# gchq/annchor

Hardware: AMD Instinct MI355X
Metric: knn_graph_builds_per_s (1 / Annchor.fit() wall-clock; BASELINE: k-NN graph build time + recall@k) (higher is better)
Workload: dtype int32 bit-vectors (Levenshtein) + f64 (bounds/regression/selection); 1 GPU; load_strings Levenshtein N=1600 n_anchors=15 k=25 p_work=0.12 niters=2; parallelism=one GPU

## Files before the change

annchor_amd/_native.py:

```python
import ctypes
import os

import numpy as np

_HERE = os.path.dirname(os.path.abspath(__file__))
LIB_PATH = os.environ.get("ANNCHOR_HIP_LIB", os.path.join(_HERE, "libannchor_hip.so"))

F_D, F_A, F_SID, F_IJS, F_I_PTR, F_I_IDX, F_FEATURES, F_NCM, F_RA, F_LABELS, F_THRESH, F_PROB, F_CAND, F_NEXT, F_DAD = range(1, 16)
_FIELD_DTYPE = {
    F_D: np.float64, F_A: np.int64, F_SID: np.uint64, F_IJS: np.int64, F_I_PTR: np.int64, F_I_IDX: np.int64,
    F_FEATURES: np.float64, F_NCM: np.uint8, F_RA: np.float64, F_LABELS: np.int64, F_THRESH: np.float64,
    F_PROB: np.float64, F_CAND: np.int64, F_NEXT: np.int64, F_DAD: np.float64,
}

METRIC_LEVENSHTEIN, METRIC_EUCLIDEAN_F32, METRIC_EUCLIDEAN_F64, METRIC_WASSERSTEIN = 1, 2, 3, 4
METRIC_COSINE_F32, METRIC_COSINE_F64 = 5, 6
METRIC_DTW_F32, METRIC_DTW_F64 = 7, 8
METRIC_FRECHET_F32, METRIC_FRECHET_F64 = 9, 10
METRIC_HAUSDORFF_F32, METRIC_HAUSDORFF_F64 = 11, 12
METRIC_ERP_F32, METRIC_ERP_F64 = 13, 14
METRIC_EMD_POINTS_F32, METRIC_EMD_POINTS_F64 = 15, 16
METRIC_JACCARD_TOKENS, METRIC_JACCARD_BITS = 17, 18
METRIC_WEIGHTED_LEVENSHTEIN = 19
METRIC_MSM_F32, METRIC_MSM_F64 = 20, 21
# ... 80 lines not shown
    "annchor_legacy_prefetch": (ctypes.c_int, [ctypes.c_uint32, _i64]),
    "annchor_legacy_generate": (ctypes.c_int, [ctypes.c_uint32, _i64]),
    "annchor_legacy_generate_at_next_wait": (ctypes.c_int, [_vp, ctypes.c_uint32, _i64, _i64]),
    "annchor_legacy_choice_ranks": (ctypes.c_int, [ctypes.c_uint32, _vp, _vp, _i32, _vp, _vp]),
    "annchor_legacy_choice_begin": (ctypes.c_int, [ctypes.c_uint32, _vp, _vp, _i32, ctypes.POINTER(_vp)]),
    "annchor_legacy_choice_end": (ctypes.c_int, [_vp, _vp, _vp]),
    "annchor_ols_bins": (ctypes.c_int, [_vp, _vp, _vp, _i64, _i32, _vp, _i32, _vp, _vp, _vp, _vp]),
    "annchor_gather_features": (ctypes.c_int, [_vp, _vp, _i64, _vp]),
    "annchor_evaluate_samples": (ctypes.c_int, [_vp, _vp, _i64, _vp]),
    "annchor_set_samples": (ctypes.c_int, [_vp, _vp, _i64, _vp]),
    "annchor_predict_merge": (ctypes.c_int, [_vp, _vp, _i32, _vp, _vp, _i32, _i32, _vp]),
    "annchor_merge_host_prediction": (ctypes.c_int, [_vp, _vp, _i32, _i32]),
    "annchor_set_labels": (ctypes.c_int, [_vp, _vp]),
    "annchor_select_candidates": (ctypes.c_int, [_vp, _i32, _i32, _vp, _vp, _i32, _i64, _i32,
                                                 ctypes.POINTER(_i64), ctypes.POINTER(_i64)]),
    "annchor_select_prepare": (ctypes.c_int, [_vp, _i32, _i32]),
    "annchor_mark_candidates": (ctypes.c_int, [_vp]),
    "annchor_refine_candidates": (ctypes.c_int, [_vp]),
    "annchor_park_refine": (ctypes.c_int, [_vp, _i32]),
    "annchor_set_refined": (ctypes.c_int, [_vp, _vp, _i64]),
    "annchor_update_bounds": (ctypes.c_int, [_vp]),
    "annchor_update_bounds_prepare": (ctypes.c_int, [_vp]),
    "annchor_overlap_stats": (ctypes.c_int, [_vp, _vp]),
    "annchor_neighbor_graph": (ctypes.c_int, [_vp, _i32, _vp, _vp]),
    "annchor_stream_bind": (ctypes.c_int, [_vp, _vp, _i64, _i32, _i64, _i32]),
    "annchor_stream_anchor_round": (ctypes.c_int, [_vp, _vp, _i32, _i32, ctypes.POINTER(_dbl), ctypes.POINTER(_i64)]),
    "annchor_stream_get_row": (ctypes.c_int, [_vp, _i64, _vp]),
    "annchor_stream_order": (ctypes.c_int, [_vp, _i32] + [ctypes.POINTER(_vp)] * 6 + [ctypes.POINTER(_i64), ctypes.POINTER(_i32),
                                                                                   ctypes.POINTER(_i32)]),
    "annchor_stream_knn": (ctypes.c_int, [_vp, _vp, _vp, _vp, _vp, _vp, _vp, _i64, _i32, _i32, _i32, _i32, _i32, _i32, _dbl, _i32, _i32, _vp,
                                          _vp, _vp, ctypes.POINTER(_i64)]),
    "annchor_stream_knn_begin": (ctypes.c_int, [_vp, _vp, _vp, _vp, _vp, _vp, _vp, _i64, _i32, _i32, _i32, _i32, _i32, _i32, _i32,
                                                ctypes.POINTER(_vp), ctypes.POINTER(_i64)]),
    "annchor_stream_knn_join": (ctypes.c_int, [_vp, _vp, _i32, ctypes.POINTER(_vp), ctypes.POINTER(_i64)]),
    "annchor_stream_join_rev_begin": (ctypes.c_int, [_vp, _vp, ctypes.POINTER(_vp), ctypes.POINTER(_vp), ctypes.POINTER(_i64)]),
    "annchor_stream_order_begin": (ctypes.c_int, [_vp, _i32, _i32, _i32, ctypes.POINTER(_vp), ctypes.POINTER(_vp), ctypes.POINTER(_i64)]),
    "annchor_stream_order_end": (ctypes.c_int, [_vp] + [ctypes.POINTER(_vp)] * 6 + [ctypes.POINTER(_i64), ctypes.POINTER(_i32),
                                                                                       ctypes.POINTER(_i32)]),
    "annchor_stream_last_counts": (ctypes.c_int, [_vp, ctypes.POINTER(_i64), ctypes.POINTER(_i64)]),
    "annchor_stream_last_kernel": (ctypes.c_int, [_vp, ctypes.POINTER(ctypes.c_int32), ctypes.POINTER(_i64)]),
    "annchor_stream_last_tile_kernels": (ctypes.c_int, [_vp, ctypes.POINTER(ctypes.c_int32), ctypes.POINTER(ctypes.c_int32)]),
    "annchor_stream_budget": (ctypes.c_int, [_i32, _dbl, _i32, ctypes.POINTER(_i32), ctypes.POINTER(_i32), ctypes.POINTER(_i32)]),
    "annchor_stream_knn_end": (ctypes.c_int, [_vp, _vp, _vp, _vp, ctypes.POINTER(_i64)]),
    "annchor_stream_knn_run": (ctypes.c_int, [_vp, _vp, _vp, _vp, _vp, _vp, _vp, _i64, _i32, _i32, _i32, _i32, _i32, _i32, _dbl, _i32, _i32,
                                               ctypes.POINTER(_i64)]),
    "annchor_stream_knn_fetch": (ctypes.c_int, [_vp, _vp, _vp, _vp]),
# ... 652 lines not shown
        self._chk(self.lib.annchor_mark_candidates(self.h))

    def refine_candidates(self):
        self._chk(self.lib.annchor_refine_candidates(self.h))

    def park_refine(self, action):
        self._chk(self.lib.annchor_park_refine(self.h, int(action)))

    def set_refined(self, exact):
        exact = _c(exact, np.float64)
        self._chk(self.lib.annchor_set_refined(self.h, _ptr(exact), len(exact)))

    def update_bounds(self):
        self._chk(self.lib.annchor_update_bounds(self.h))

    def update_bounds_prepare(self):
        self._chk(self.lib.annchor_update_bounds_prepare(self.h))

    def overlap_stats(self):
        out = np.zeros(2, dtype=np.int64)
        self._chk(self.lib.annchor_overlap_stats(self.h, _ptr(out)))
        return bool(out[0]), int(out[1])

    def neighbor_graph(self, k):
        idx = np.zeros((self.nx, k), dtype=np.int64)
        dist = np.zeros((self.nx, k), dtype=np.float64)
        self._chk(self.lib.annchor_neighbor_graph(self.h, int(k), _ptr(idx), _ptr(dist)))
        return idx, dist

    def stream_bind(self, X, global_base=0, device_ptr=None, shape=None):
        if device_ptr is not None:
            n, d = shape
            self._chk(self.lib.annchor_stream_bind(self.h, device_ptr, int(n), int(d), int(global_base), 1))
        else:
            X = _c(X, np.float32)
            n, d = X.shape
            self._chk(self.lib.annchor_stream_bind(self.h, _ptr(X), n, d, int(global_base), 0))
        self.nx, self.metric = int(n), METRIC_EUCLIDEAN_F32
        self._stream_dim = int(d)

    def stream_bind_f64(self, X, global_base=0, centre=None):
        X = _c(X, np.float64)
        n, d = X.shape
        cin = _c(centre, np.float64) if centre is not None else None
        if cin is not None and cin.shape != (d,):
            raise ValueError("centre must be float64 [%d]" % d)
# ... 361 lines not shown
```

annchor_amd/csrc/common.h:

```cpp
#pragma once
#include <hip/hip_runtime.h>

#include <cstdint>
#include <cstdio>
#include <cstring>
#include <string>
#include <vector>
#include <chrono>

#include "../../include/annchor_hip.h"

#define ANN_WAVE 64

struct DevBuf {
    void *p = nullptr;
    size_t cap = 0;
    bool in_arena = false;
    template <typename T> T *as() const { return reinterpret_cast<T *>(p); }
};

struct ProfEntry {
    const char *name;
    double ms = 0;
    int64_t launches = 0;
// ... 105 lines not shown

    DevBuf lb, ub, dad, RA, prob;
    DevBuf anc, ncm, label;
    bool have_features = false, have_RA = false;
    int64_t n_unc = -1;
    int64_t n_unc_after_features = -1;

    DevBuf spos, sy;
    DevBuf draw_J, draw_next, draw_q1;
    DevBuf sfeat, spred;
    int64_t sfeat_rows = 0;
    DevBuf model;
    DevBuf ols_scratch;
    std::vector<DevBuf *> own_allocs;
    int prof_group_entry = -1;
    bool model_fitted = false;
    bool errs_on_device = false;
    int model_nb = 0;
    DevBuf dev_flags;
    bool dev_flags_clean = false;
    bool gn_err_clean = false;
    bool state_prewarmed = false;
    DevBuf sstats;
    DevBuf hs_key, hs_pos, hs_misc;
    int64_t nsamp = 0;

    DevBuf thresh;
    DevBuf cand, next;
    int64_t ncand = 0, nnext = 0;
    bool cand_marked = false;
    DevBuf gl_val, gl_pos, gl_cnt, gl_ncomp, marked, markcount;
    DevBuf gn_state;
    bool sel_prepared = false;
    int sel_k = 0, sel_nmin = 0;
    bool gn_pending = false;
    int gn_round = 0, gn_L = 0;
    DevBuf sel_hist, sel_state, blk_cnt, blk_off;
    DevBuf sel_pass_state;
    DevBuf tie_lists, tie_hist;
    const void *tie_hist_clean = nullptr;
    DevBuf sel2, sel_bufA, sel_bufB, sel_seg;
    const void *sel2_clean = nullptr;
    DevBuf errs, errptr;
    DevBuf ecdf_index;
    DevBuf cptr, cidx, cval;
    DevBuf c16, cbnd;
// ... 31 lines not shown
        }                                                                                       \
    } while (0)

#define ANN_TRY(expr)                \
    do {                             \
        int _r = (expr);             \
        if (_r != ANNCHOR_OK) return _r; \
    } while (0)

#define ANN_REQUIRE(c, cond, code, ...)    \
    do {                                   \
        if (!(cond)) {                     \
            ann_set_err((c), __VA_ARGS__); \
            return (code);                 \
        }                                  \
    } while (0)

int ann_reserve(annchor_ctx *c, DevBuf &b, size_t bytes);
int ann_arena_init(annchor_ctx *c, int64_t nx);
int ann_prewarm_state(annchor_ctx *c);
void ann_lev_ap_probe(annchor_ctx *c);
size_t ann_sel2_table_bytes();
size_t ann_tie_hist_bytes();
size_t ann_sel_state_bytes();
int ann_h2d(annchor_ctx *c, void *dst, const void *src, size_t bytes);
hipError_t ann_sync(annchor_ctx *c, const char *where);
int ann_dev_alloc(annchor_ctx *c, void **p, size_t want, size_t *got);
void ann_dev_free(annchor_ctx *c, void *p, size_t bytes);
struct Sel2Epilogue;
int ann_kth_async(annchor_ctx *c, const double *vals, const uint8_t *flag, int64_t n, const int64_t *ks, int nk,
                  const unsigned long long **d_prefix, const int **d_unfinished, const Sel2Epilogue *epi = nullptr);
void ann_kth_async_done(annchor_ctx *c);
int ann_d2h(annchor_ctx *c, void *dst, const void *src, size_t bytes);
int ann_d2h_then(annchor_ctx *c, void *dst, const void *src, size_t bytes, int (*then)(annchor_ctx *));
int ann_d2h2(annchor_ctx *c, void *dst1, const void *src1, size_t bytes1, void *dst2, const void *src2, size_t bytes2);

int ann_prof_entry(annchor_ctx *c, const char *name);
struct ProfGroup {
    annchor_ctx *c;
    int entry = -1;
    hipEvent_t a = nullptr, b = nullptr;
    ProfGroup(annchor_ctx *ctx, const char *name);
    ~ProfGroup();
};

struct ProfScope {
// ... 172 lines not shown
```

annchor_amd/csrc/ctx.hip:

```cpp
#include <cstdarg>
#include <cmath>
#include <cstdlib>

#include "common.h"
#include <algorithm>
#include <chrono>
#include <mutex>

static std::string g_create_err;
void ann_stream_release(annchor_ctx *c);
void ann_enemies_release(annchor_ctx *c);
void ann_draw_forget(annchor_ctx *c);
void ann_comm_release(annchor_ctx *c);
hipError_t ann_comm_guarded_sync(annchor_ctx *c, hipStream_t stream, const char *where);

const char *ann_set_err(annchor_ctx *c, const char *fmt, ...)
{
    char buf[1024];
    va_list ap;
    va_start(ap, fmt);
    vsnprintf(buf, sizeof buf, fmt, ap);
    va_end(ap);
    if (c && c->comm_aborted && c->err.rfind("collective timed out", 0) == 0) return c->err.c_str();
    if (c) c->err = buf; else g_create_err = buf;
// ... 127 lines not shown
    size_t bytes = (size_t)(pairs * 112.0) + (size_t)nx * 4096 + ((size_t)64 << 20);
    if (c->arena) {
        if (c->arena_size >= bytes || c->arena_off != 0) return ANNCHOR_OK;
        ann_dev_free(c, c->arena, c->arena_size);
        c->arena = nullptr;
        c->arena_size = 0;
    }
    void *p = nullptr;
    size_t got = 0;
    if ((p = pool_take(c->device, bytes, &got)) != nullptr) bytes = got;
    else if (hipMalloc(&p, bytes) != hipSuccess) { (void)hipGetLastError(); return ANNCHOR_OK; }
    c->arena = (char *)p;
    c->arena_size = bytes;
    c->arena_off = 0;
    return ANNCHOR_OK;
}

int ann_prewarm_state(annchor_ctx *c)
{
    if (!c->arena || c->state_prewarmed) return ANNCHOR_OK;
    const size_t slot_bytes = sizeof(unsigned long long) * 4 * 1024 + 64;
    struct Piece { DevBuf *b; size_t bytes; };
    Piece pieces[] = {{&c->dev_flags, sizeof(int32_t) * 16}, {&c->lev_cursors, 4 * sizeof(int32_t)}, {&c->sel_state, ann_sel_state_bytes()},
                      {&c->sel2, ann_sel2_table_bytes()},    {&c->tie_hist, ann_tie_hist_bytes()},   {&c->lev_ap, slot_bytes}};
    size_t need = 0;
    for (auto &q : pieces) {
        if (q.b->p) return ANNCHOR_OK;
        need += (q.bytes + 255) & ~(size_t)255;
    }
    if (c->arena_off + need > c->arena_size) return ANNCHOR_OK;
    char *first = c->arena + c->arena_off;
    for (auto &q : pieces) ANN_TRY(ann_reserve(c, *q.b, q.bytes));
    ANN_CHECK_HIP(c, hipMemsetAsync(first, 0, need, c->stream));
    c->dev_flags_clean = true;
    c->lev_cursor_epoch = 0;
    c->gn_err_clean = true;
    c->sel2_clean = c->sel2.p;
    c->tie_hist_clean = c->tie_hist.p;
    c->lev_ap_epoch = 0;
    c->state_prewarmed = true;
    return ANNCHOR_OK;
}

int ann_h2d(annchor_ctx *c, void *dst, const void *src, size_t bytes)
{
    if (bytes == 0) return ANNCHOR_OK;
    if (c->pin && bytes <= annchor_ctx::PIN_SLOT_BYTES) {
        const int sl = c->pin_next;
        c->pin_next = (sl + 1) % annchor_ctx::PIN_SLOTS;
        if (c->pin_busy[sl]) ANN_CHECK_HIP(c, hipEventSynchronize(c->pin_ev[sl]));
        unsigned char *slot = c->pin + (size_t)sl * annchor_ctx::PIN_SLOT_BYTES;
        memcpy(slot, src, bytes);
        ANN_CHECK_HIP(c, hipMemcpyAsync(dst, slot, bytes, hipMemcpyHostToDevice, c->stream));
        ANN_CHECK_HIP(c, hipEventRecord(c->pin_ev[sl], c->stream));
        c->pin_busy[sl] = true;
        return ANNCHOR_OK;
    }
    ANN_CHECK_HIP(c, hipMemcpyAsync(dst, src, bytes, hipMemcpyHostToDevice, c->stream));
    ANN_CHECK_HIP(c, ann_sync(c, __func__));
    return ANNCHOR_OK;
}
// ... 227 lines not shown
}

int ann_side_join(annchor_ctx *c)
{
    if (!c->side_pending) return ANNCHOR_OK;
    c->side_pending = false;
    ANN_CHECK_HIP(c, hipStreamWaitEvent(c->main_stream, c->side_done_ev, 0));
    return ANNCHOR_OK;
}

SideScope::SideScope(annchor_ctx *ctx) : c(ctx) { c->stream = c->side_stream; }
SideScope::~SideScope()
{
    (void)hipEventRecord(c->side_done_ev, c->side_stream);
    c->side_pending = true;
    c->stream = c->main_stream;
}

extern "C" int annchor_overlap_stats(annchor_ctx *c, int64_t *out)
{
    if (!c || !out) return ANNCHOR_EINVAL;
    out[0] = c->overlap_parts != 0 && c->side_stream != nullptr;
    out[1] = c->ub_prepared_taken;
    return ANNCHOR_OK;
}

extern "C" int annchor_create(int device, annchor_ctx **out)
{
    if (!out) return ANNCHOR_EINVAL;
    *out = nullptr;
    int count = 0;
    hipError_t e = hipGetDeviceCount(&count);
    if (e != hipSuccess || count <= 0) {
        ann_set_err(nullptr, "no HIP device available (%s)", e == hipSuccess ? "count = 0" : hipGetErrorString(e));
        return ANNCHOR_ENODEV;
    }
    if (device < 0 || device >= count) {
        ann_set_err(nullptr, "device %d out of range (have %d)", device, count);
        return ANNCHOR_EINVAL;
    }
    annchor_ctx *c = new annchor_ctx();
    c->device = device;
    if ((e = hipSetDevice(device)) != hipSuccess) {
        ann_set_err(nullptr, "device init failed: %s", hipGetErrorString(e));
        delete c;
        return ANNCHOR_EHIP;
// ... 961 lines not shown
```

annchor_amd/csrc/features.hip:

```cpp
#include "common.h"
#include "selstate.h"
#include <mutex>

#pragma clang fp contract(off)

__global__ __launch_bounds__(256) void k_features(const int2 *__restrict__ ij, int64_t n, const double *__restrict__ Dt,
                                                 int64_t nx, int na, const int32_t *__restrict__ cA,
                                                 const int32_t *__restrict__ anchorRank, double *__restrict__ lb,
                                                 double *__restrict__ ub, double *__restrict__ dad,
                                                 uint8_t *__restrict__ anc, uint8_t *__restrict__ ncm)
{
    int64_t p = (int64_t)blockIdx.x * blockDim.x + threadIdx.x;
    if (p >= n) return;
    const int2 q = ij[p];
    const int i = q.x, j = q.y;
    double l = 0.0, u = INFINITY;
    const int i0 = __builtin_amdgcn_readfirstlane(i);
    if (__all(i == i0)) {
        for (int a0 = 0; a0 < na; a0 += 8) {
            double di[8], dj[8];
#pragma unroll
            for (int e = 0; e < 8; ++e) {
                const size_t row = (size_t)min(a0 + e, na - 1) * nx;
                di[e] = Dt[row + i0];
// ... 416 lines not shown
    }
    __syncthreads();
    if ((int)threadIdx.x < be.nb) {
        unsigned long long s = 0;
        for (int w = 0; w < BC_THREADS / 64; ++w) s += lc[w][threadIdx.x];
        if (s) atomicAdd(&counts[threadIdx.x], s);
    }
}
__global__ __launch_bounds__(BC_THREADS) void k_bin_counts(const double *__restrict__ dad, const uint8_t *__restrict__ ncm,
                                                          int64_t n, BinEdges be, unsigned long long *__restrict__ counts)
{
    bin_counts_body(dad, ncm, n, be, counts);
}

__global__ __launch_bounds__(BC_THREADS) void k_bin_counts_dev(const double *__restrict__ dad, const uint8_t *__restrict__ ncm,
                                                              int64_t n, SamplerStats *__restrict__ st)
{
    __shared__ BinEdges be;
    if (threadIdx.x == 0) be = st->be;
    __syncthreads();
    bin_counts_body(dad, ncm, n, be, st->counts);
}

static int load_bins(annchor_ctx *c, const double *bins, int32_t nbins, BinEdges &be);

__host__ __device__ __forceinline__ unsigned long long ann_splitmix64(unsigned long long x)
{
    x += 0x9E3779B97F4A7C15ull;
    x = (x ^ (x >> 30)) * 0xBF58476D1CE4E5B9ull;
    x = (x ^ (x >> 27)) * 0x94D049BB133111EBull;
    return x ^ (x >> 31);
}

#define HS_CAP 4096
struct HsParams {
    unsigned long long seed_key;
    unsigned long long thr[MAXBINS];
};

#define HS_U 8
__global__ __launch_bounds__(256) void k_hs_collect(const double *__restrict__ dad, const uint8_t *__restrict__ ncm, int64_t n,
                                                   BinEdges be, HsParams hp, unsigned long long *__restrict__ lkey,
                                                   int32_t *__restrict__ lpos, uint32_t *__restrict__ lcnt)
{
    __shared__ double se[MAXBINS + 1];
    __shared__ unsigned long long sthr[MAXBINS];
// ... 166 lines not shown
    for (int k = 0; k <= nbins; ++k) be.e[k] = bins[k];
    return ANNCHOR_OK;
}

extern "C" int annchor_bin_counts(annchor_ctx *c, const double *bins, int32_t nbins, int64_t *counts)
{
    if (!c || !bins || !counts) return ANNCHOR_EINVAL;
    ANN_REQUIRE(c, c->have_features, ANNCHOR_EINVAL, "features not computed");
    ANN_CHECK_HIP(c, hipSetDevice(c->device));
    BinEdges be;
    ANN_TRY(load_bins(c, bins, nbins, be));
    ANN_TRY(ann_reserve(c, c->tmp2, 8 * MAXBINS));
    ANN_CHECK_HIP(c, hipMemsetAsync(c->tmp2.p, 0, 8 * MAXBINS, c->stream));
    const int64_t ntiles = (c->n + BC_TILE - 1) / BC_TILE;
    const int blocks = (int)(ntiles <= 256 ? ntiles : std::min<int64_t>(1024, std::max<int64_t>(256, ntiles / 4)));
    {
        ProfScope ps(c, "sampler_bin_counts", (double)c->n * 9.0);
        k_bin_counts<<<blocks, BC_THREADS, 0, c->stream>>>(c->dad.as<double>(), c->ncm.as<uint8_t>(), c->n, be,
                                                   c->tmp2.as<unsigned long long>());
    }
    return ann_d2h(c, counts, c->tmp2.p, 8 * (size_t)nbins);
}

extern "C" int annchor_sampler_stats(annchor_ctx *c, const int64_t *ks, int32_t n_partitions, double *q, double *edges,
                                     int64_t *counts, int32_t *fused)
{
    if (!c || !ks || !q || !edges || !counts || !fused) return ANNCHOR_EINVAL;
    ANN_REQUIRE(c, c->have_features, ANNCHOR_EINVAL, "features not computed");
    ANN_REQUIRE(c, n_partitions >= 2 && n_partitions <= MAXBINS, ANNCHOR_ELIMIT, "2..%d partitions supported", MAXBINS);
    ANN_CHECK_HIP(c, hipSetDevice(c->device));
    *fused = 0;
    const unsigned long long *d_prefix = nullptr;
    const int *d_unfinished = nullptr;
    ANN_TRY(ann_reserve(c, c->sstats, sizeof(SamplerStats)));
    SamplerStats *st = c->sstats.as<SamplerStats>();
    {
        Sel2Epilogue ep;
        memset(&ep, 0, sizeof ep);
        ep.kind = 1; ep.st = st; ep.nparts = n_partitions;
        ANN_TRY(ann_kth_async(c, c->dad.as<double>(), c->ncm.as<uint8_t>(), c->n, ks, 2, &d_prefix, &d_unfinished, &ep));
    }
    if (d_prefix) {
        const int64_t ntiles = (c->n + BC_TILE - 1) / BC_TILE;
        const int blocks = (int)(ntiles <= 256 ? ntiles : std::min<int64_t>(1024, std::max<int64_t>(256, ntiles / 4)));
        {
            ProfScope ps(c, "sampler_bin_counts", (double)c->n * 9.0);
            k_bin_counts_dev<<<blocks, BC_THREADS, 0, c->stream>>>(c->dad.as<double>(), c->ncm.as<uint8_t>(), c->n, st);
        }
        ANN_CHECK_HIP(c, hipGetLastError());
        SamplerStats h;
        if (c->park_refine) {
            c->park_refine = false;
            ANN_TRY(ann_d2h_then(c, &h, st, sizeof h, ann_refine_released));
        } else
        ANN_TRY(ann_d2h(c, &h, st, sizeof h));
        const int unfinished = h.unfinished;
        ann_kth_async_done(c);
        if (!unfinished) {
            q[0] = h.q[0]; q[1] = h.q[1];
            for (int b = 0; b <= n_partitions; ++b) edges[b] = h.be.e[b];
            for (int b = 0; b < n_partitions; ++b) counts[b] = (int64_t)h.counts[b];
            *fused = 1;
            return ANNCHOR_OK;
        }
    }
    return ann_kth_smallest(c, c->dad.as<double>(), c->ncm.as<uint8_t>(), c->n, ks, 2, q);
}

#define RB_THREADS 256
#define RB_ITEMS 8
#define RB_TILE (RB_THREADS * RB_ITEMS)

__global__ __launch_bounds__(RB_THREADS) void k_rb_count(const double *__restrict__ dad, const uint8_t *__restrict__ ncm,
                                                        int64_t n, BinEdges be, uint32_t *__restrict__ blkcnt)
{
    __shared__ unsigned int lc[MAXBINS];
    for (int t = threadIdx.x; t < MAXBINS; t += blockDim.x) lc[t] = 0;
    __syncthreads();
    int64_t base = (int64_t)blockIdx.x * RB_TILE;
    double v[RB_ITEMS];
// ... 1084 lines not shown
```

annchor_amd/csrc/scan.hip:

```cpp
#include "common.h"
#include "selstate.h"

#define SCAN_THREADS 256
#define SCAN_ITEMS 8
#define SCAN_TILE (SCAN_THREADS * SCAN_ITEMS)

__device__ __forceinline__ int64_t block_exclusive_scan_i64(int64_t v, int64_t *total)
{
    __shared__ int64_t wsum[SCAN_THREADS / 64];
    const int lane = threadIdx.x & 63, wave = threadIdx.x >> 6;
    int64_t inc = v;
#pragma unroll
    for (int off = 1; off < 64; off <<= 1) {
        int64_t o = __shfl_up(inc, off);
        if (lane >= off) inc += o;
    }
    if (lane == 63) wsum[wave] = inc;
    __syncthreads();
    int64_t base = 0, tot = 0;
#pragma unroll
    for (int w = 0; w < SCAN_THREADS / 64; ++w) {
        if (w < wave) base += wsum[w];
        tot += wsum[w];
    }
// ... 175 lines not shown
        if (threadIdx.x == 0) { o->nq = nq; o->vor = st_prev->vor; o->vand = st_prev->vand; }
    }
    if (pass == 8) return;
    const int shift = 56 - 8 * pass;
    if ((((st_prev->vor ^ st_prev->vand) >> shift) & 0xffull) == 0) return;
    uint32_t *hist = hist_all + (size_t)pass * SEL_MAXQ * 256;
    for (int t = threadIdx.x; t < SEL_MAXQ * 256; t += blockDim.x) lh[t] = 0;
    uint64_t pre[SEL_MAXQ];
    for (int q = 0; q < SEL_MAXQ; ++q) pre[q] = q < nq ? sh.prefix[q] : 0;
    __syncthreads();
    const uint64_t himask = shift == 56 ? 0ull : (~0ull << (shift + 8));
    for (int64_t t = (int64_t)blockIdx.x * blockDim.x + threadIdx.x; t < n; t += (int64_t)gridDim.x * blockDim.x) {
        if (flag && !flag[t]) continue;
        uint64_t key = ann_key_asc(vals[t]);
        uint32_t d = (uint32_t)(key >> shift) & 0xffu;
        for (int q = 0; q < nq; ++q)
            if ((key & himask) == (pre[q] & himask)) atomicAdd(&lh[q * 256 + d], 1u);
    }
    __syncthreads();
    for (int t = threadIdx.x; t < nq * 256; t += blockDim.x)
        if (lh[t]) atomicAdd(&hist[t], lh[t]);
}

#define S2_T 1024
#define S2_ITEMS 8
#define S2_TILE (S2_T * S2_ITEMS)
#define S2_MAXWG 1024
#define S2_NB0 2048
#define S2_NB1 2048
#define S2_NB2 1024
#define S2_NB3 2048
#define S2_CAP 4096
#define S3_SAMPLE_MIN (1ll << 23)
#define S2_LEVEL3_MIN (1ll << 22)
struct Sel2State {
    uint64_t prefix[SEL_MAXQ];
    int64_t k[SEL_MAXQ];
    int nq, unfinished;
    unsigned long long cnt;
};
struct Sel3Info {
    uint64_t lo[SEL_MAXQ], hi[SEL_MAXQ];
    long long lt[SEL_MAXQ], eq[SEL_MAXQ];
    long long drop[SEL_MAXQ];
    long long kept;
};
struct Sel2Tables {
    uint32_t hist0[S2_NB0];
    uint32_t hist1[SEL_MAXQ * S2_NB1];
    uint32_t hist2[SEL_MAXQ * S2_NB2];
    uint32_t hist3[SEL_MAXQ * S2_NB3];
    unsigned long long vor[2][SEL_MAXQ], vnand[2][SEL_MAXQ];
    Sel2State st1, st2, st3, out;
    Sel3Info s3;
    uint64_t skey[8192];
    uint32_t sdone;
};
#define S2_ZERO_BYTES offsetof(Sel2Tables, st1)
struct Sel2Sh {
    uint32_t wsum[S2_T / 64];
    int digit;
    int64_t krem;
};

template <int NB> __device__ __forceinline__ void sel2_step(const uint32_t *hist, int64_t k_in, Sel2Sh &sh, int &digit, int64_t &krem)
{
    constexpr int PER = NB >= S2_T ? NB / S2_T : 1;
    const int tid = threadIdx.x, lane = tid & 63, wave = tid >> 6;
    uint32_t cb[PER], s = 0;
#pragma unroll
    for (int j = 0; j < PER; ++j) { cb[j] = tid * PER + j < NB ? hist[tid * PER + j] : 0u; s += cb[j]; }
    uint32_t inc = s;
#pragma unroll
    for (int off = 1; off < 64; off <<= 1) {
        uint32_t o = __shfl_up(inc, off);
        if (lane >= off) inc += o;
    }
    __syncthreads();
    if (lane == 63) sh.wsum[wave] = inc;
    if (tid == 0) { sh.digit = NB - 1; sh.krem = 0; }
    __syncthreads();
    uint32_t base = 0, total = 0;
    for (int w = 0; w < S2_T / 64; ++w) { const uint32_t x = sh.wsum[w]; if (w < wave) base += x; total += x; }
    int64_t k = k_in;
    if (k >= (int64_t)total) k = (int64_t)total - 1;
    int64_t ex = (int64_t)base + inc - s;
    if (s != 0 && k >= ex && k < ex + s) {
#pragma unroll
        for (int j = 0; j < PER; ++j) {
            if (k >= ex && k < ex + cb[j]) { sh.digit = tid * PER + j; sh.krem = k - ex; }
            ex += cb[j];
        }
    }
    __syncthreads();
    digit = sh.digit;
    krem = sh.krem;
}

__global__ __launch_bounds__(S2_T) void k_sel2_hist0(const double *__restrict__ vals, const uint8_t *__restrict__ flag, int64_t n,
                                                    Sel2Tables *__restrict__ tb, const uint32_t *__restrict__ segcnt)
{
    __shared__ uint32_t lh[S2_NB0];
    for (int t = threadIdx.x; t < S2_NB0; t += S2_T) lh[t] = 0;
    __syncthreads();
    const int lane = threadIdx.x & 63;
    const int64_t ntiles = (n + S2_TILE - 1) / S2_TILE;
    for (int64_t tile = blockIdx.x; tile < ntiles; tile += gridDim.x) {
        const uint32_t lim = segcnt ? segcnt[tile] : (uint32_t)S2_TILE;
        if (lim == 0) break;
        double v[S2_ITEMS];
        uint8_t f[S2_ITEMS];
#pragma unroll
        for (int j = 0; j < S2_ITEMS; ++j) {
            const int64_t t = tile * S2_TILE + j * S2_T + threadIdx.x;
            v[j] = ann_ldc(vals, t, n);
            f[j] = flag ? ann_ldc(flag, t, n) : (uint8_t)1;
            if (t >= n || (uint32_t)(j * S2_T + threadIdx.x) >= lim) f[j] = 0;
        }
#pragma unroll
        for (int j = 0; j < S2_ITEMS; ++j) {
            const bool act = f[j] != 0;
// ... 686 lines not shown
```

annchor_amd/csrc/selstate.h:

```cpp
#pragma once
#include "common.h"

struct BinEdges {
    double e[MAXBINS + 1];
    int nb;
};

struct SamplerStats {
    BinEdges be;
    double q[2];
    unsigned long long counts[MAXBINS];
    int unfinished;
};

struct CutState {
    double t1, t5;
    int64_t K1, K5;
    int64_t e1, e5;
    int64_t ncand, nnext;
    int all1, all5;
    unsigned long long rk1, rk5;
    int64_t tie_n1, tie_n5;
    int64_t tie_gt1, tie_gt5;
    long long tie_bin1, tie_bin5;
    long long tie_rem1, tie_rem5;
    long long tie_len1, tie_len5;
    int64_t tie_got1, tie_got5;
    int tie_overflow;
    int sel_unfinished;
};

struct Sel2Epilogue {
    int kind;
    SamplerStats *st;
    int nparts;
    CutState *cs;
    CutState cs_init;
    int need1, need5, force_redo;
};

__device__ __forceinline__ void sel2_epilogue(const Sel2Epilogue &ep, const uint64_t *prefix , int unfinished)
{
    if (ep.kind == 1) {
        SamplerStats *st = ep.st;
        const int nparts = ep.nparts;
        const double q1 = ann_key_asc_inv(prefix[0]), q3 = ann_key_asc_inv(prefix[1]);
        st->q[0] = q1; st->q[1] = q3;
        const int num = nparts - 1, div = num > 1 ? num - 1 : 1;
        const double delta = q3 - q1, step = delta / (double)div;
        st->be.nb = nparts;
        st->be.e[0] = -INFINITY;
        for (int i = 0; i < num; ++i) {
            double y;
            if (step != 0.0) { const double p = (double)i * step; y = p + q1; }
            else { const double p = ((double)i / (double)div) * delta; y = p + q1; }
            if (num > 1 && i == num - 1) y = q3;
            st->be.e[1 + i] = y;
        }
        st->be.e[nparts] = INFINITY;
        for (int b = 0; b < MAXBINS; ++b) st->counts[b] = 0;
        st->unfinished = unfinished;
    } else if (ep.kind == 2) {
        CutState init = ep.cs_init;
// ... 8 lines not shown
```

include/annchor_hip.h:

```cpp
#ifndef ANNCHOR_HIP_H
#define ANNCHOR_HIP_H

#include <stdint.h>

#ifdef __cplusplus
extern "C" {
#endif

typedef struct annchor_ctx annchor_ctx;

enum {
    ANNCHOR_OK = 0,
    ANNCHOR_EINVAL = -1,
    ANNCHOR_EHIP = -2,
    ANNCHOR_ENODEV = -3,
    ANNCHOR_ELIMIT = -4,
    ANNCHOR_ESTATE = -5
};

enum { ANNCHOR_METRIC_NONE = 0, ANNCHOR_METRIC_LEVENSHTEIN = 1, ANNCHOR_METRIC_EUCLIDEAN_F32 = 2,
       ANNCHOR_METRIC_EUCLIDEAN_F64 = 3, ANNCHOR_METRIC_WASSERSTEIN = 4, ANNCHOR_METRIC_COSINE_F32 = 5,
       ANNCHOR_METRIC_COSINE_F64 = 6, ANNCHOR_METRIC_DTW_F32 = 7, ANNCHOR_METRIC_DTW_F64 = 8,
       ANNCHOR_METRIC_FRECHET_F32 = 9, ANNCHOR_METRIC_FRECHET_F64 = 10, ANNCHOR_METRIC_HAUSDORFF_F32 = 11,
       ANNCHOR_METRIC_HAUSDORFF_F64 = 12, ANNCHOR_METRIC_ERP_F32 = 13, ANNCHOR_METRIC_ERP_F64 = 14,
// ... 149 lines not shown
                                       int64_t *ranks_out, int32_t *taken);
int annchor_download_samples(annchor_ctx *ctx, int64_t *positions, double *feats, double *sample_y, double *sample_predict);
int annchor_fit_regression_device(annchor_ctx *ctx, const double *bins, int32_t nbins, int32_t first_iteration, int32_t is_metric);
int annchor_fit_errors_device(annchor_ctx *ctx);
int annchor_model_download(annchor_ctx *ctx, double *W, double *c, int32_t *status, int64_t *err_ptr, int32_t *flags );
int annchor_errors_download(annchor_ctx *ctx, double *errs, int64_t n_errs);
int annchor_model_download_with_errors(annchor_ctx *ctx, double *W, double *c, int32_t *status, int64_t *err_ptr, int32_t *flags ,
                                       double *errs, int64_t errs_cap, int64_t *n_errs);

int annchor_select_candidates(annchor_ctx *ctx, int32_t n_neighbors, int32_t nmin, const double *errs,
                              const int64_t *err_ptr, int32_t nlabels, int64_t n_refine,
                              int32_t lookahead, int64_t *n_cand, int64_t *n_next);
int annchor_select_prepare(annchor_ctx *ctx, int32_t n_neighbors, int32_t nmin);
int annchor_mark_candidates(annchor_ctx *ctx);
int annchor_refine_candidates(annchor_ctx *ctx);
int annchor_lev_persist_state(int set);

int annchor_park_refine(annchor_ctx *ctx, int32_t action);
int annchor_set_refined(annchor_ctx *ctx, const double *exact, int64_t n_cand);

int annchor_update_bounds(annchor_ctx *ctx);
int annchor_update_bounds_prepare(annchor_ctx *ctx);
int annchor_overlap_stats(annchor_ctx *ctx, int64_t *out);

int annchor_neighbor_graph(annchor_ctx *ctx, int32_t n_neighbors, int64_t *ng_idx, double *ng_dist);

int annchor_stream_bind(annchor_ctx *ctx, const float *X, int64_t n_local, int32_t dim, int64_t global_base,
                        int32_t x_on_device);
int annchor_stream_anchor_round(annchor_ctx *ctx, const float *anchor_vec, int32_t round, int32_t n_anchors,
                                double *local_max, int64_t *local_arg);
int annchor_stream_get_row(annchor_ctx *ctx, int64_t local_idx, float *out);
int annchor_stream_order(annchor_ctx *ctx, int32_t min_tiles, void **Xs, void **rs, void **perm, void **lo, void **hi,
                         void **mid, int64_t *n_pad, int32_t *n_tiles, int32_t *dim_padded);
int annchor_stream_order_begin(annchor_ctx *ctx, int32_t min_tiles, int32_t tile_begin, int32_t tile_count, void **order_local,
                               void **order_all, int64_t *order_bytes);
int annchor_stream_order_end(annchor_ctx *ctx, void **Xs, void **rs, void **perm, void **lo, void **hi, void **mid, int64_t *n_pad,
                             int32_t *n_tiles, int32_t *dim_padded);
int annchor_stream_knn(annchor_ctx *ctx, const void *Xs_all, const void *rs_all, const void *perm_all, const void *lo_all,
                       const void *hi_all, const void *mid_all, int64_t n_all, int32_t nt_all, int32_t n_anchors, int32_t dim_padded,
                       int32_t tile_begin, int32_t tile_count, int32_t k, double p_work, int32_t join_passes, int32_t join_extra,
                       int64_t *row_ids, int64_t *ng_idx, double *ng_dist, int64_t *tile_evals);
int annchor_stream_knn_run(annchor_ctx *ctx, const void *Xs_all, const void *rs_all, const void *perm_all, const void *lo_all,
                           const void *hi_all, const void *mid_all, int64_t n_all, int32_t nt_all, int32_t n_anchors,
                           int32_t dim_padded, int32_t tile_begin, int32_t tile_count, int32_t k, double p_work, int32_t join_passes,
                           int32_t join_extra, int64_t *tile_evals);
int annchor_stream_knn_fetch(annchor_ctx *ctx, int64_t *row_ids, int64_t *ng_idx, double *ng_dist);
// ... 89 lines not shown
```

Measured before the change: 384.7 graphs/s.

## Add dense half-integer histogram route for Levenshtein sampler statistics

For Levenshtein metrics with short strings, sampler statistics now come from one dense 8192-bin histogram of doubled anchor-distance values, built with wave-aggregated shared atomics. A single-block finish kernel then selects both quantiles and redistributes bin counts into the sampler partitions. This replaces the multi-pass radix k-th selection followed by a separate bin-count pass. If any value is not a half-integer in range, the result is flagged unfinished and the code falls back to the original route, at the cost of one wasted pass in that case.

New measurement: 384.8 graphs/s, median of 4. No clear change (+0.0%).

```diff
diff --git a/annchor_amd/_native.py b/annchor_amd/_native.py
--- a/annchor_amd/_native.py
+++ b/annchor_amd/_native.py
@@ -126,6 +126,7 @@
     "annchor_update_bounds": (ctypes.c_int, [_vp]),
     "annchor_update_bounds_prepare": (ctypes.c_int, [_vp]),
     "annchor_overlap_stats": (ctypes.c_int, [_vp, _vp]),
+    "annchor_sampler_route_stats": (ctypes.c_int, [_vp, _vp]),
     "annchor_neighbor_graph": (ctypes.c_int, [_vp, _i32, _vp, _vp]),
     "annchor_stream_bind": (ctypes.c_int, [_vp, _vp, _i64, _i32, _i64, _i32]),
     "annchor_stream_anchor_round": (ctypes.c_int, [_vp, _vp, _i32, _i32, ctypes.POINTER(_dbl), ctypes.POINTER(_i64)]),
@@ -824,6 +825,11 @@
         self._chk(self.lib.annchor_overlap_stats(self.h, _ptr(out)))
         return bool(out[0]), int(out[1])
 
+    def sampler_route_stats(self):
+        out = np.zeros(2, dtype=np.int64)
+        self._chk(self.lib.annchor_sampler_route_stats(self.h, _ptr(out)))
+        return int(out[0]), int(out[1])
+
     def neighbor_graph(self, k):
         idx = np.zeros((self.nx, k), dtype=np.int64)
         dist = np.zeros((self.nx, k), dtype=np.float64)
diff --git a/annchor_amd/csrc/common.h b/annchor_amd/csrc/common.h
--- a/annchor_amd/csrc/common.h
+++ b/annchor_amd/csrc/common.h
@@ -151,6 +151,9 @@
     bool gn_err_clean = false;
     bool state_prewarmed = false;
     DevBuf sstats;
+    DevBuf stats_hist;
+    const void *stats_hist_clean = nullptr;
+    int64_t stats_hist_taken = 0, stats_hist_fell = 0;
     DevBuf hs_key, hs_pos, hs_misc;
     int64_t nsamp = 0;
 
@@ -228,6 +231,7 @@
 void ann_lev_ap_probe(annchor_ctx *c);
 size_t ann_sel2_table_bytes();
 size_t ann_tie_hist_bytes();
+size_t ann_stats_hist_bytes();
 size_t ann_sel_state_bytes();
 int ann_h2d(annchor_ctx *c, void *dst, const void *src, size_t bytes);
 hipError_t ann_sync(annchor_ctx *c, const char *where);
diff --git a/annchor_amd/csrc/ctx.hip b/annchor_amd/csrc/ctx.hip
--- a/annchor_amd/csrc/ctx.hip
+++ b/annchor_amd/csrc/ctx.hip
@@ -173,7 +173,8 @@
     const size_t slot_bytes = sizeof(unsigned long long) * 4 * 1024 + 64;
     struct Piece { DevBuf *b; size_t bytes; };
     Piece pieces[] = {{&c->dev_flags, sizeof(int32_t) * 16}, {&c->lev_cursors, 4 * sizeof(int32_t)}, {&c->sel_state, ann_sel_state_bytes()},
-                      {&c->sel2, ann_sel2_table_bytes()},    {&c->tie_hist, ann_tie_hist_bytes()},   {&c->lev_ap, slot_bytes}};
+                      {&c->sel2, ann_sel2_table_bytes()},    {&c->tie_hist, ann_tie_hist_bytes()},   {&c->lev_ap, slot_bytes},
+                      {&c->stats_hist, ann_stats_hist_bytes()}};
     size_t need = 0;
     for (auto &q : pieces) {
         if (q.b->p) return ANNCHOR_OK;
@@ -188,6 +189,7 @@
     c->gn_err_clean = true;
     c->sel2_clean = c->sel2.p;
     c->tie_hist_clean = c->tie_hist.p;
+    c->stats_hist_clean = c->stats_hist.p;
     c->lev_ap_epoch = 0;
     c->state_prewarmed = true;
     return ANNCHOR_OK;
@@ -461,6 +463,14 @@
     if (!c || !out) return ANNCHOR_EINVAL;
     out[0] = c->overlap_parts != 0 && c->side_stream != nullptr;
     out[1] = c->ub_prepared_taken;
+    return ANNCHOR_OK;
+}
+
+extern "C" int annchor_sampler_route_stats(annchor_ctx *c, int64_t *out)
+{
+    if (!c || !out) return ANNCHOR_EINVAL;
+    out[0] = c->stats_hist_taken;
+    out[1] = c->stats_hist_fell;
     return ANNCHOR_OK;
 }
 
diff --git a/annchor_amd/csrc/features.hip b/annchor_amd/csrc/features.hip
--- a/annchor_amd/csrc/features.hip
+++ b/annchor_amd/csrc/features.hip
@@ -462,6 +462,97 @@
     bin_counts_body(dad, ncm, n, be, st->counts);
 }
 
+#define SH_BINS 8192
+#define SH_ITEMS 8
+#define SH_TILE (S2_T * SH_ITEMS)
+size_t ann_stats_hist_bytes() { return sizeof(unsigned long long) * (SH_BINS + 1); }
+
+__global__ __launch_bounds__(S2_T) void k_stats_hist(const double *__restrict__ dad, const uint8_t *__restrict__ ncm, int64_t n,
+                                                    unsigned long long *__restrict__ tab)
+{
+    __shared__ uint32_t lh[SH_BINS];
+    __shared__ int bad;
+    for (int t = threadIdx.x; t < SH_BINS; t += S2_T) lh[t] = 0;
+    if (threadIdx.x == 0) bad = 0;
+    __syncthreads();
+    const int lane = threadIdx.x & 63;
+    bool mybad = false;
+    const int64_t ntiles = (n + SH_TILE - 1) / SH_TILE;
+    for (int64_t tile = blockIdx.x; tile < ntiles; tile += gridDim.x) {
+        double v[SH_ITEMS];
+        uint8_t f[SH_ITEMS];
+#pragma unroll
+        for (int j = 0; j < SH_ITEMS; ++j) {
+            const int64_t t = tile * SH_TILE + j * S2_T + threadIdx.x;
+            v[j] = ann_ldc(dad, t, n);
+            f[j] = ann_ldc(ncm, t, n);
+            if (t >= n) f[j] = 0;
+        }
+#pragma unroll
+        for (int j = 0; j < SH_ITEMS; ++j) {
+            const double h = v[j] + v[j];
+            const bool ok = __double_as_longlong(h) >= 0 && h < (double)SH_BINS && h == floor(h);
+            mybad |= f[j] != 0 && !ok;
+            const bool act = f[j] != 0 && ok;
+            const uint32_t d = act ? (uint32_t)(int)h : 0u;
+            const unsigned long long am = __ballot(act);
+            if (!am) continue;
+            const int lead = __ffsll((long long)am) - 1;
+            const uint32_t d0 = __shfl(d, lead);
+            const unsigned long long m = __ballot(act && d == d0);
+            if (lane == lead) atomicAdd(&lh[d0], (uint32_t)__popcll(m));
+            if (act && d != d0) atomicAdd(&lh[d], 1u);
+        }
+    }
+    if (mybad) bad = 1;
+    __syncthreads();
+    for (int t = threadIdx.x; t < SH_BINS; t += S2_T)
+        if (lh[t]) atomicAdd(&tab[t], (unsigned long long)lh[t]);
+    if (threadIdx.x == 0 && bad) atomicAdd(&tab[SH_BINS], 1ull);
+}
+
+__global__ __launch_bounds__(S2_T) void k_stats_finish(unsigned long long *__restrict__ tab, int64_t k0, int64_t k1, Sel2Epilogue ep)
+{
+    constexpr int PER = SH_BINS / S2_T;
+    __shared__ uint32_t lh[SH_BINS];
+    __shared__ Sel2Sh sh;
+    __shared__ SamplerStats sst;
+    static_assert(sizeof(SamplerStats) % sizeof(unsigned long long) == 0, "SamplerStats is copied in 8-byte words");
+    const int tid = threadIdx.x;
+    unsigned long long cb[PER];
+#pragma unroll
+    for (int j = 0; j < PER; ++j) { cb[j] = tab[tid * PER + j]; lh[tid * PER + j] = (uint32_t)cb[j]; }
+    const bool violated = tid == 0 && tab[SH_BINS] != 0;
+#pragma unroll
+    for (int j = 0; j < PER; ++j)
+        if (cb[j]) tab[tid * PER + j] = 0;
+    if (tid == 0 && violated) tab[SH_BINS] = 0;
+    __syncthreads();
+    int d0, d1;
+    int64_t krem;
+    sel2_step<SH_BINS>(lh, k0, sh, d0, krem);
+    sel2_step<SH_BINS>(lh, k1, sh, d1, krem);
+    if (tid == 0) {
+        uint32_t total = 0;
+        for (int w = 0; w < S2_T / 64; ++w) total += sh.wsum[w];
+        const uint64_t prefix[2] = {ann_key_asc((double)d0 * 0.5), ann_key_asc((double)d1 * 0.5)};
+        Sel2Epilogue lep;
+        lep.kind = 1; lep.st = &sst; lep.nparts = ep.nparts;
+        sel2_epilogue(lep, prefix, (violated || total == 0) ? 1 : 0);
+    }
+    __syncthreads();
+#pragma unroll
+    for (int j = 0; j < PER; ++j)
+        if (cb[j]) {
+            const int b = sampler_bin(sst.be, (double)(tid * PER + j) * 0.5);
+            if (b >= 0) atomicAdd(&sst.counts[b], cb[j]);
+        }
+    __syncthreads();
+    const unsigned long long *src = reinterpret_cast<const unsigned long long *>(&sst);
+    unsigned long long *dst = reinterpret_cast<unsigned long long *>(ep.st);
+    for (int t = tid; t < (int)(sizeof(SamplerStats) / sizeof(unsigned long long)); t += S2_T) dst[t] = src[t];
+}
+
 static int load_bins(annchor_ctx *c, const double *bins, int32_t nbins, BinEdges &be);
 
 __host__ __device__ __forceinline__ unsigned long long ann_splitmix64(unsigned long long x)
@@ -674,6 +765,13 @@
     return ann_d2h(c, counts, c->tmp2.p, 8 * (size_t)nbins);
 }
 
+static bool stats_hist_wanted(const annchor_ctx *c)
+{
+    const char *e = getenv("ANNCHOR_STATS_HIST");
+    if (e && *e) return atoi(e) != 0;
+    return c->metric == ANNCHOR_METRIC_LEVENSHTEIN && c->maxlen < SH_BINS / 2;
+}
+
 extern "C" int annchor_sampler_stats(annchor_ctx *c, const int64_t *ks, int32_t n_partitions, double *q, double *edges,
                                      int64_t *counts, int32_t *fused)
 {
@@ -682,20 +780,30 @@
     ANN_REQUIRE(c, n_partitions >= 2 && n_partitions <= MAXBINS, ANNCHOR_ELIMIT, "2..%d partitions supported", MAXBINS);
     ANN_CHECK_HIP(c, hipSetDevice(c->device));
     *fused = 0;
-    const unsigned long long *d_prefix = nullptr;
-    const int *d_unfinished = nullptr;
     ANN_TRY(ann_reserve(c, c->sstats, sizeof(SamplerStats)));
     SamplerStats *st = c->sstats.as<SamplerStats>();
-    {
-        Sel2Epilogue ep;
-        memset(&ep, 0, sizeof ep);
-        ep.kind = 1; ep.st = st; ep.nparts = n_partitions;
-        ANN_TRY(ann_kth_async(c, c->dad.as<double>(), c->ncm.as<uint8_t>(), c->n, ks, 2, &d_prefix, &d_unfinished, &ep));
-    }
-    if (d_prefix) {
-        const int64_t ntiles = (c->n + BC_TILE - 1) / BC_TILE;
-        const int blocks = (int)(ntiles <= 256 ? ntiles : std::min<int64_t>(1024, std::max<int64_t>(256, ntiles / 4)));
-        {
+    Sel2Epilogue ep;
+    memset(&ep, 0, sizeof ep);
+    ep.kind = 1; ep.st = st; ep.nparts = n_partitions;
+    for (int route = stats_hist_wanted(c) ? 0 : 1; route < 2; ++route) {
+        if (route == 0) {
+            ANN_TRY(ann_reserve(c, c->stats_hist, ann_stats_hist_bytes()));
+            if (c->stats_hist_clean != c->stats_hist.p) {
+                ANN_CHECK_HIP(c, hipMemsetAsync(c->stats_hist.p, 0, ann_stats_hist_bytes(), c->stream));
+                c->stats_hist_clean = c->stats_hist.p;
+            }
+            const int64_t ntiles = (c->n + SH_TILE - 1) / SH_TILE;
+            const int grid = (int)(ntiles <= 256 ? ntiles : std::min<int64_t>(1024, std::max<int64_t>(256, ntiles / 4)));
+            ProfScope ps(c, "sampler_stats_hist", (double)c->n * 9.0);
+            k_stats_hist<<<grid, S2_T, 0, c->stream>>>(c->dad.as<double>(), c->ncm.as<uint8_t>(), c->n, c->stats_hist.as<unsigned long long>());
+            k_stats_finish<<<1, S2_T, 0, c->stream>>>(c->stats_hist.as<unsigned long long>(), ks[0], ks[1], ep);
+        } else {
+            const unsigned long long *d_prefix = nullptr;
+            const int *d_unfinished = nullptr;
+            ANN_TRY(ann_kth_async(c, c->dad.as<double>(), c->ncm.as<uint8_t>(), c->n, ks, 2, &d_prefix, &d_unfinished, &ep));
+            if (!d_prefix) break;
+            const int64_t ntiles = (c->n + BC_TILE - 1) / BC_TILE;
+            const int blocks = (int)(ntiles <= 256 ? ntiles : std::min<int64_t>(1024, std::max<int64_t>(256, ntiles / 4)));
             ProfScope ps(c, "sampler_bin_counts", (double)c->n * 9.0);
             k_bin_counts_dev<<<blocks, BC_THREADS, 0, c->stream>>>(c->dad.as<double>(), c->ncm.as<uint8_t>(), c->n, st);
         }
@@ -707,7 +815,8 @@
         } else
         ANN_TRY(ann_d2h(c, &h, st, sizeof h));
         const int unfinished = h.unfinished;
-        ann_kth_async_done(c);
+        if (route == 1) ann_kth_async_done(c);
+        else ++(unfinished ? c->stats_hist_fell : c->stats_hist_taken);
         if (!unfinished) {
             q[0] = h.q[0]; q[1] = h.q[1];
             for (int b = 0; b <= n_partitions; ++b) edges[b] = h.be.e[b];
diff --git a/annchor_amd/csrc/scan.hip b/annchor_amd/csrc/scan.hip
--- a/annchor_amd/csrc/scan.hip
+++ b/annchor_amd/csrc/scan.hip
@@ -221,7 +221,6 @@
         if (lh[t]) atomicAdd(&hist[t], lh[t]);
 }
 
-#define S2_T 1024
 #define S2_ITEMS 8
 #define S2_TILE (S2_T * S2_ITEMS)
 #define S2_MAXWG 1024
@@ -256,46 +255,6 @@
     uint32_t sdone;
 };
 #define S2_ZERO_BYTES offsetof(Sel2Tables, st1)
-struct Sel2Sh {
-    uint32_t wsum[S2_T / 64];
-    int digit;
-    int64_t krem;
-};
-
-template <int NB> __device__ __forceinline__ void sel2_step(const uint32_t *hist, int64_t k_in, Sel2Sh &sh, int &digit, int64_t &krem)
-{
-    constexpr int PER = NB >= S2_T ? NB / S2_T : 1;
-    const int tid = threadIdx.x, lane = tid & 63, wave = tid >> 6;
-    uint32_t cb[PER], s = 0;
-#pragma unroll
-    for (int j = 0; j < PER; ++j) { cb[j] = tid * PER + j < NB ? hist[tid * PER + j] : 0u; s += cb[j]; }
-    uint32_t inc = s;
-#pragma unroll
-    for (int off = 1; off < 64; off <<= 1) {
-        uint32_t o = __shfl_up(inc, off);
-        if (lane >= off) inc += o;
-    }
-    __syncthreads();
-    if (lane == 63) sh.wsum[wave] = inc;
-    if (tid == 0) { sh.digit = NB - 1; sh.krem = 0; }
-    __syncthreads();
-    uint32_t base = 0, total = 0;
-    for (int w = 0; w < S2_T / 64; ++w) { const uint32_t x = sh.wsum[w]; if (w < wave) base += x; total += x; }
-    int64_t k = k_in;
-    if (k >= (int64_t)total) k = (int64_t)total - 1;
-    int64_t ex = (int64_t)base + inc - s;
-    if (s != 0 && k >= ex && k < ex + s) {
-#pragma unroll
-        for (int j = 0; j < PER; ++j) {
-            if (k >= ex && k < ex + cb[j]) { sh.digit = tid * PER + j; sh.krem = k - ex; }
-            ex += cb[j];
-        }
-    }
-    __syncthreads();
-    digit = sh.digit;
-    krem = sh.krem;
-}
-
 __global__ __launch_bounds__(S2_T) void k_sel2_hist0(const double *__restrict__ vals, const uint8_t *__restrict__ flag, int64_t n,
                                                     Sel2Tables *__restrict__ tb, const uint32_t *__restrict__ segcnt)
 {
diff --git a/annchor_amd/csrc/selstate.h b/annchor_amd/csrc/selstate.h
--- a/annchor_amd/csrc/selstate.h
+++ b/annchor_amd/csrc/selstate.h
@@ -39,6 +39,47 @@
     int need1, need5, force_redo;
 };
 
+#define S2_T 1024
+struct Sel2Sh {
+    uint32_t wsum[S2_T / 64];
+    int digit;
+    int64_t krem;
+};
+
+template <int NB> __device__ __forceinline__ void sel2_step(const uint32_t *hist, int64_t k_in, Sel2Sh &sh, int &digit, int64_t &krem)
+{
+    constexpr int PER = NB >= S2_T ? NB / S2_T : 1;
+    const int tid = threadIdx.x, lane = tid & 63, wave = tid >> 6;
+    uint32_t cb[PER], s = 0;
+#pragma unroll
+    for (int j = 0; j < PER; ++j) { cb[j] = tid * PER + j < NB ? hist[tid * PER + j] : 0u; s += cb[j]; }
+    uint32_t inc = s;
+#pragma unroll
+    for (int off = 1; off < 64; off <<= 1) {
+        uint32_t o = __shfl_up(inc, off);
+        if (lane >= off) inc += o;
+    }
+    __syncthreads();
+    if (lane == 63) sh.wsum[wave] = inc;
+    if (tid == 0) { sh.digit = NB - 1; sh.krem = 0; }
+    __syncthreads();
+    uint32_t base = 0, total = 0;
+    for (int w = 0; w < S2_T / 64; ++w) { const uint32_t x = sh.wsum[w]; if (w < wave) base += x; total += x; }
+    int64_t k = k_in;
+    if (k >= (int64_t)total) k = (int64_t)total - 1;
+    int64_t ex = (int64_t)base + inc - s;
+    if (s != 0 && k >= ex && k < ex + s) {
+#pragma unroll
+        for (int j = 0; j < PER; ++j) {
+            if (k >= ex && k < ex + cb[j]) { sh.digit = tid * PER + j; sh.krem = k - ex; }
+            ex += cb[j];
+        }
+    }
+    __syncthreads();
+    digit = sh.digit;
+    krem = sh.krem;
+}
+
 __device__ __forceinline__ void sel2_epilogue(const Sel2Epilogue &ep, const uint64_t *prefix , int unfinished)
 {
     if (ep.kind == 1) {
diff --git a/include/annchor_hip.h b/include/annchor_hip.h
--- a/include/annchor_hip.h
+++ b/include/annchor_hip.h
@@ -195,6 +195,7 @@
 int annchor_update_bounds(annchor_ctx *ctx);
 int annchor_update_bounds_prepare(annchor_ctx *ctx);
 int annchor_overlap_stats(annchor_ctx *ctx, int64_t *out);
+int annchor_sampler_route_stats(annchor_ctx *ctx, int64_t *out);
 
 int annchor_neighbor_graph(annchor_ctx *ctx, int32_t n_neighbors, int64_t *ng_idx, double *ng_dist);
 
```
